# dayae1204/WeCLIP-ViT-CoMer

Hardware: AMD Instinct MI355X
Metric: images/sec (train fwd+bwd) ViT-B/16 512x512 VOC (higher is better)
Workload: dtype f16 MFMA operands / f32 accumulate, f32 residual+softmax+LN, PAR f32 arithmetic on 16-bit fixed-point affinities (precision=fast); 1 GPU; WeCLIP VOC full train step (the reference's model: frozen CLIP ViT-B/16 + adapters + decoder + GradCAM/affinity/PAR pseudo-labels), batch 16/GPU at 512x512, K=2 classes/image (BASELINE configs[2] without the ViT-CoMer inserts, for which the reference has no code); global_batch=16, parallelism=dp1

## Files before the change

### weclip-vit-comer_amd/csrc/par.hip

```cpp
#include "common.h"
#include <stdlib.h>

#define PAR_MAX_TAPS 64

struct ParTaps {
    int n;
    int dy[PAR_MAX_TAPS];
    int dx[PAR_MAX_TAPS];
    float pi[PAR_MAX_TAPS];
};

__device__ __forceinline__ int clampi(int v, int hi) { return v < 0 ? 0 : (v > hi ? hi : v); }

__global__ __launch_bounds__(256) void par_affinity_kernel(const float* __restrict__ img,
                                                            float* __restrict__ aff, int H, int W,
                                                            float w1, ParTaps taps) {
    const int x = blockIdx.x * 64 + (threadIdx.x & 63);
    const int y = blockIdx.y * 4 + (threadIdx.x >> 6);
    if (x >= W || y >= H) return;
    const long HW = (long)H * W;
    const float* I = img + (long)blockIdx.z * 3 * HW;
    const long p = (long)y * W + x;
    const float c0 = I[p], c1 = I[HW + p], c2 = I[2 * HW + p];
    const int T = taps.n;
    float s0 = 0.f, s1 = 0.f, s2 = 0.f;
    for (int t = 0; t < T; ++t) {
        const long o = (long)clampi(y + taps.dy[t], H - 1) * W + clampi(x + taps.dx[t], W - 1);
        s0 += I[o]; s1 += I[HW + o]; s2 += I[2 * HW + o];
    }
    const float m0 = s0 / T, m1 = s1 / T, m2 = s2 / T;
    float q0 = 0.f, q1 = 0.f, q2 = 0.f;
    for (int t = 0; t < T; ++t) {
        const long o = (long)clampi(y + taps.dy[t], H - 1) * W + clampi(x + taps.dx[t], W - 1);
        const float a = I[o] - m0, b = I[HW + o] - m1, c = I[2 * HW + o] - m2;
        q0 += a * a; q1 += b * b; q2 += c * c;
    }
    const float d0 = sqrtf(q0 / (T - 1)) + 1e-8f, d1 = sqrtf(q1 / (T - 1)) + 1e-8f,
                d2 = sqrtf(q2 / (T - 1)) + 1e-8f;
    float mx = -INFINITY, sum = 0.f;
    for (int t = 0; t < T; ++t) {
        const long o = (long)clampi(y + taps.dy[t], H - 1) * W + clampi(x + taps.dx[t], W - 1);
        const float a = fabsf(I[o] - c0) / d0 / w1, b = fabsf(I[HW + o] - c1) / d1 / w1,
                    c = fabsf(I[2 * HW + o] - c2) / d2 / w1;
        const float e = -(a * a + b * b + c * c) / 3.0f;
        const float nm = fmaxf(mx, e);
        sum = sum * __expf(mx - nm) + __expf(e - nm);
        mx = nm;
    }
    const float inv = 1.0f / sum;
    float* A = aff + (long)blockIdx.z * T * HW + p;
    for (int t = 0; t < T; ++t) {
        const long o = (long)clampi(y + taps.dy[t], H - 1) * W + clampi(x + taps.dx[t], W - 1);
        const float a = fabsf(I[o] - c0) / d0 / w1, b = fabsf(I[HW + o] - c1) / d1 / w1,
                    c = fabsf(I[2 * HW + o] - c2) / d2 / w1;
        const float e = -(a * a + b * b + c * c) / 3.0f;
        A[(long)t * HW] = __expf(e - mx) * inv + taps.pi[t];
    }
}

__device__ __forceinline__ long aff_base(bool tiled, long img, int T, int H, int W, int y, int x, long* tstride) {
    if (tiled) {
        const int XT = (W + 63) >> 6;
        *tstride = 64;
        return ((img * H + y) * XT + (x >> 6)) * (long)T * 64 + (x & 63);
    }
    *tstride = (long)H * W;
    return img * T * (long)H * W + (long)y * W + x;
}

#define PAR_Q_SLOTS(T_) ((T_) / 2 + 1)
template <int ND, bool TILED, bool H16 = false>
__global__ __launch_bounds__(256) void par_affinity_reg_kernel(const float* __restrict__ img,
                                                                float* __restrict__ aff, int H, int W,
                                                                float w1, ParTaps taps) {
    constexpr int T = 8 * ND;
    const int x = blockIdx.x * 64 + (threadIdx.x & 63);
    const int y = blockIdx.y * 4 + (threadIdx.x >> 6);
    if (x >= W || y >= H) return;
    const long HW = (long)H * W;
    const float* I = img + (long)blockIdx.z * 3 * HW;
    const long p = (long)y * W + x;
    const float c0 = I[p], c1 = I[HW + p], c2 = I[2 * HW + p];
    float v0[T], v1[T], v2[T];
    float s0 = 0.f, s1 = 0.f, s2 = 0.f;
    constexpr int RY[8] = {0, 0, 0, 1, 1, 2, 2, 2}, CX[8] = {0, 1, 2, 0, 2, 0, 1, 2};
#pragma unroll
    for (int dl = 0; dl < ND; ++dl) {
        const int d = taps.dx[8 * dl + 2];
        const int rw[3] = {clampi(y - d, H - 1) * W, y * W, clampi(y + d, H - 1) * W};
        const int cl[3] = {clampi(x - d, W - 1), x, clampi(x + d, W - 1)};
#pragma unroll
        for (int u = 0; u < 8; ++u) {
            const int t = 8 * dl + u;
            const int o = rw[RY[u]] + cl[CX[u]];
            v0[t] = I[o]; v1[t] = I[HW + o]; v2[t] = I[2 * HW + o];
            s0 += v0[t]; s1 += v1[t]; s2 += v2[t];
        }
    }
    const float m0 = s0 / T, m1 = s1 / T, m2 = s2 / T;
    float q0 = 0.f, q1 = 0.f, q2 = 0.f;
#pragma unroll
    for (int t = 0; t < T; ++t) {
        const float a = v0[t] - m0, b = v1[t] - m1, c = v2[t] - m2;
        q0 += a * a; q1 += b * b; q2 += c * c;
    }
    const float d0 = sqrtf(q0 / (T - 1)) + 1e-8f, d1 = sqrtf(q1 / (T - 1)) + 1e-8f,
                d2 = sqrtf(q2 / (T - 1)) + 1e-8f;
    const float r0 = 1.0f / (d0 * w1), r1 = 1.0f / (d1 * w1), r2 = 1.0f / (d2 * w1);
    float mx = -INFINITY;
#pragma unroll
    for (int t = 0; t < T; ++t) {
        const float a = fabsf(v0[t] - c0) * r0, b = fabsf(v1[t] - c1) * r1, c = fabsf(v2[t] - c2) * r2;
        v0[t] = -(a * a + b * b + c * c) * (1.0f / 3.0f);
        mx = fmaxf(mx, v0[t]);
    }
    float sum = 0.f;
#pragma unroll
    for (int t = 0; t < T; ++t) {
        v0[t] = __expf(v0[t] - mx);
        sum += v0[t];
    }
    const float inv = 1.0f / sum;
    if constexpr (H16) {
        const int XT = (W + 63) >> 6;
        unsigned* A2 = reinterpret_cast<unsigned*>(aff) + (((long)blockIdx.z * H + y) * XT + (x >> 6)) * (long)PAR_Q_SLOTS(T) * 64 + (x & 63);
        float amax = 0.f;
#pragma unroll
        for (int t = 0; t < T; ++t) {
            v0[t] = v0[t] * inv + taps.pi[t];
            amax = fmaxf(amax, v0[t]);
        }
        const float scale = amax * (1.0f / 65535.0f), rs = 65535.0f / amax;
        float carry = 0.f;
#pragma unroll
        for (int j = 0; j < T / 2; ++j) {
            const float a0 = v0[2 * j] + carry;
            const float q0 = fminf(fmaxf(rintf(a0 * rs), 0.f), 65535.f);
            carry = a0 - q0 * scale;
            const float a1 = v0[2 * j + 1] + carry;
            const float q1 = fminf(fmaxf(rintf(a1 * rs), 0.f), 65535.f);
            carry = a1 - q1 * scale;
            A2[j * 64] = (unsigned)q0 | ((unsigned)q1 << 16);
        }
        A2[(T / 2) * 64] = __float_as_uint(scale);
        return;
    }
    long ts;
    float* A = aff + aff_base(TILED, blockIdx.z, T, H, W, y, x, &ts);
#pragma unroll
    for (int t = 0; t < T; ++t) A[t * ts] = v0[t] * inv + taps.pi[t];
}

static void launch_affinity(const float* img, float* aff, int nb, int H, int W, const ParTaps& tp,
                            hipStream_t st, bool tiled, bool h16 = false) {
    dim3 grid(wc_cdiv(W, 64), wc_cdiv(H, 4), nb);
    const int pr = wc_prof_begin(st);
    if (tp.n == 48 && tiled && h16) {
        hipLaunchKernelGGL((par_affinity_reg_kernel<6, true, true>), grid, dim3(256), 0, st, img, aff, H, W, 0.3f, tp);
        wc_prof_end(pr, "par_affinity_reg_kernel<6, true, true>", 4.0 * nb * (double)H * W * 3 + nb * (double)H * W * (2.0 * tp.n + 4.0), st);
        return;
    }
    if (tp.n == 48 && tiled)
        hipLaunchKernelGGL((par_affinity_reg_kernel<6, true>), grid, dim3(256), 0, st, img, aff, H, W, 0.3f, tp);
    else if (tp.n == 48)
        hipLaunchKernelGGL((par_affinity_reg_kernel<6, false>), grid, dim3(256), 0, st, img, aff, H, W, 0.3f, tp);
    else
        hipLaunchKernelGGL(par_affinity_kernel, grid, dim3(256), 0, st, img, aff, H, W, 0.3f, tp);
    wc_prof_end(pr, tp.n == 48 ? (tiled ? "par_affinity_reg_kernel<6, true>" : "par_affinity_reg_kernel<6, false>") : "par_affinity_kernel",
                4.0 * nb * (double)H * W * (3 + tp.n), st);
}

#ifndef PAR_TAP_BATCH
#define PAR_TAP_BATCH 8
#endif
template <int CG, bool TILED, bool H16 = false, int ROWS = 4, int PAR_HALO = 4>
__global__ __launch_bounds__(64 * ROWS) void par_iter_kernel(const float* __restrict__ aff,
                                                        const float* __restrict__ min,
                                                        float* __restrict__ mout, int C, int H,
                                                        int W, ParTaps taps) {
    constexpr int TW = 64 + 2 * PAR_HALO, TH = ROWS + 2 * PAR_HALO;
    __shared__ float tile[H16 ? CG * TH * TW : 1];
    const int lx = threadIdx.x & 63, ly = threadIdx.x >> 6;
    int x = blockIdx.x * 64 + lx;
    int y = blockIdx.y * ROWS + ly;
    const bool live = x < W && y < H;
    if constexpr (H16) {
        x = x < W ? x : W - 1;
        y = y < H ? y : H - 1;
    } else {
        if (!live) return;
    }
    const long HW = (long)H * W;
    const long p = (long)y * W + x;
    const int T = taps.n;
    long ts;
    const float* A = aff + aff_base(TILED, blockIdx.z, T, H, W, y, x, &ts);
    const unsigned* A2 = reinterpret_cast<const unsigned*>(aff) +
                         (((long)blockIdx.z * H + y) * ((W + 63) >> 6) + (x >> 6)) * (long)PAR_Q_SLOTS(T) * 64 + (x & 63);
    float qscale = 1.f;
    if constexpr (H16) qscale = __uint_as_float(A2[(T / 2) * 64]);
    const float* M = min + (long)blockIdx.z * C * HW;
    float* O = mout + (long)blockIdx.z * C * HW + p;
    for (int cb = 0; cb < C; cb += CG) {
        float acc[CG];
        const float* Mc[CG];
#pragma unroll
        for (int k = 0; k < CG; ++k) {
            acc[k] = 0.f;
            Mc[k] = M + (long)(cb + k < C ? cb + k : C - 1) * HW;
        }
        if constexpr (H16) {
            if (cb) __syncthreads();
            for (int ty = ly; ty < TH; ty += ROWS) {
                const int ro = clampi(blockIdx.y * ROWS + ty - PAR_HALO, H - 1) * W;
                for (int tx = lx; tx < TW; tx += 64) {
                    const unsigned ob = (unsigned)(ro + clampi(blockIdx.x * 64 + tx - PAR_HALO, W - 1)) * 4u;
#pragma unroll
                    for (int k = 0; k < CG; ++k)
                        tile[(k * TH + ty) * TW + tx] = *reinterpret_cast<const float*>(reinterpret_cast<const char*>(Mc[k]) + ob);
                }
            }
            __syncthreads();
        }
        constexpr int TB_ = PAR_TAP_BATCH;
        int t = 0;
        for (; t + TB_ <= T; t += TB_) {
            float a[TB_], m[TB_][CG];
            unsigned a2[TB_ / 2];
            if constexpr (H16) {
#pragma unroll
                for (int u = 0; u < TB_ / 2; ++u) a2[u] = A2[((t >> 1) + u) * 64];
            }
            bool near = false;
            if constexpr (H16) near = (taps.dy[t] < 0 ? -taps.dy[t] : taps.dy[t]) <= PAR_HALO && (taps.dx[t] < 0 ? -taps.dx[t] : taps.dx[t]) <= PAR_HALO;
            if (near) {
                const int tb = (ly + PAR_HALO) * TW + lx + PAR_HALO;
#pragma unroll
                for (int u = 0; u < TB_; ++u) {
                    const int o = tb + (taps.dy[t + u] * TW + taps.dx[t + u]);
#pragma unroll
                    for (int k = 0; k < CG; ++k) m[u][k] = tile[k * TH * TW + o];
                }
            } else if constexpr (H16) {
                const int d = taps.dx[t + 2];
                const int rw[3] = {clampi(y - d, H - 1) * W, y * W, clampi(y + d, H - 1) * W};
                const int cl[3] = {clampi(x - d, W - 1), x, clampi(x + d, W - 1)};
                constexpr int RY[8] = {0, 0, 0, 1, 1, 2, 2, 2}, CX[8] = {0, 1, 2, 0, 2, 0, 1, 2};
                static_assert(TB_ == 8, "one batch = one dilation");
#pragma unroll
                for (int u = 0; u < TB_; ++u) {
                    const unsigned ob = (unsigned)(rw[RY[u]] + cl[CX[u]]) * 4u;
#pragma unroll
                    for (int k = 0; k < CG; ++k) m[u][k] = *reinterpret_cast<const float*>(reinterpret_cast<const char*>(Mc[k]) + ob);
                }
            } else {
#pragma unroll
                for (int u = 0; u < TB_; ++u) {
                    a[u] = A[(t + u) * ts];
                    const int o = clampi(y + taps.dy[t + u], H - 1) * W + clampi(x + taps.dx[t + u], W - 1);
#pragma unroll
                    for (int k = 0; k < CG; ++k) m[u][k] = Mc[k][o];
                }
            }
            if constexpr (H16) {
#pragma unroll
                for (int u = 0; u < TB_ / 2; ++u) {
                    a[2 * u] = (float)(a2[u] & 0xffffu);
                    a[2 * u + 1] = (float)(a2[u] >> 16);
                }
            }
#pragma unroll
            for (int u = 0; u < TB_; ++u)
#pragma unroll
                for (int k = 0; k < CG; ++k) acc[k] = fmaf(a[u], m[u][k], acc[k]);
        }
        for (; t < T; ++t) {
            const float a = A[t * ts];
            const int o = clampi(y + taps.dy[t], H - 1) * W + clampi(x + taps.dx[t], W - 1);
#pragma unroll
            for (int k = 0; k < CG; ++k) acc[k] = fmaf(a, Mc[k][o], acc[k]);
        }
#pragma unroll
        for (int k = 0; k < CG; ++k)
            if (cb + k < C && live) O[(long)(cb + k) * HW] = H16 ? acc[k] * qscale : acc[k];
    }
}

__global__ __launch_bounds__(256) void par_labels_kernel(const float* __restrict__ masks,
                                                          const long* __restrict__ valid_key,
                                                          const int* __restrict__ nch,
                                                          long* __restrict__ labels, int C, long HW) {
    const long p = (long)blockIdx.x * 256 + threadIdx.x;
    if (p >= HW) return;
    const int b = blockIdx.y;
    const int n = nch ? nch[b] : C;
    const float* M = masks + (long)b * C * HW + p;
    float best = M[0];
    int bi = 0;
    for (int c = 1; c < n; ++c) {
        const float v = M[(long)c * HW];
        if (v > best) { best = v; bi = c; }
    }
    labels[(long)b * HW + p] = valid_key[(long)b * C + bi];
}

static int build_taps(ParTaps* tp, const int* dilations, int n_dil, float w1, float w2) {
    if (!dilations || n_dil < 1 || n_dil * 8 > PAR_MAX_TAPS) return 1;
    static const int DY[8] = {-1, -1, -1, 0, 0, 1, 1, 1};
    static const int DX[8] = {-1, 0, 1, -1, 1, -1, 0, 1};
    const int T = n_dil * 8;
    float pos[PAR_MAX_TAPS];
    for (int d = 0; d < n_dil; ++d)
        for (int k = 0; k < 8; ++k) {
            const int t = d * 8 + k;
            tp->dy[t] = DY[k] * dilations[d];
            tp->dx[t] = DX[k] * dilations[d];
            pos[t] = (float)dilations[d] * ((DY[k] != 0 && DX[k] != 0) ? sqrtf(2.0f) : 1.0f);
        }
    float mean = 0.f;
    for (int t = 0; t < T; ++t) mean += pos[t];
    mean /= T;
    float var = 0.f;
    for (int t = 0; t < T; ++t) var += (pos[t] - mean) * (pos[t] - mean);
    const float sd = sqrtf(var / (T - 1)) + 1e-8f;
    float e[PAR_MAX_TAPS], mx = -INFINITY, sum = 0.f;
    for (int t = 0; t < T; ++t) {
        const float v = pos[t] / sd / w1;
        e[t] = -(v * v);
        mx = fmaxf(mx, e[t]);
    }
    for (int t = 0; t < T; ++t) sum += expf(e[t] - mx);
    for (int t = 0; t < T; ++t) tp->pi[t] = w2 * expf(e[t] - mx) / sum;
    tp->n = T;
    return 0;
}

extern "C" int wc_par_affinity(const float* img, float* aff, int B, int H, int W,
                               const int* dilations, int n_dil, void* stream) {
    WC_CHECK_ARG(img && aff && B > 0 && H > 0 && W > 0, "wc_par_affinity: bad argument");
    ParTaps tp;
    WC_CHECK_ARG(build_taps(&tp, dilations, n_dil, 0.3f, 0.01f) == 0, "wc_par_affinity: 1..8 dilations");
    launch_affinity(img, aff, B, H, W, tp, (hipStream_t)stream, false);
    WC_LAUNCH_CHECK("par_affinity_kernel");
    return WC_OK;
}

static const char* par_iter_name(int C, bool tiled, bool h16) {
    static const char* hn[3] = {"par_iter_kernel<2, true, true, 8, 12>", "par_iter_kernel<3, true, true, 8, 12>", "par_iter_kernel<4, true, true, 8, 12>"};
    static const char* names[2][3] = {{"par_iter_kernel<2, false>", "par_iter_kernel<3, false>", "par_iter_kernel<4, false>"},
                                      {"par_iter_kernel<2, true>", "par_iter_kernel<3, true>", "par_iter_kernel<4, true>"}};
    const int ci = C <= 2 ? 0 : (C == 3 ? 1 : 2);
    return h16 ? hn[ci] : names[tiled ? 1 : 0][ci];
}
static double par_iter_bytes(int B, int C, int H, int W, const ParTaps& tp, bool h16) {
    return h16 ? B * (double)H * W * (2.0 * tp.n + 4.0 + 8.0 * C) : 4.0 * B * (double)H * W * (tp.n + 2 * C);
}

static int launch_iter(const float* aff, const float* src, float* dst, int B, int C, int H, int W,
                       const ParTaps& tp, hipStream_t st, bool tiled, bool h16 = false, bool prof = true) {
    dim3 grid(wc_cdiv(W, 64), wc_cdiv(H, 4), B);
    if (h16) {
        const int pr = prof ? wc_prof_begin(st) : -1;
        dim3 grid8(wc_cdiv(W, 64), wc_cdiv(H, 8), B);
        if (C <= 2) hipLaunchKernelGGL((par_iter_kernel<2, true, true, 8, 12>), grid8, dim3(512), 0, st, aff, src, dst, C, H, W, tp);
        else if (C == 3) hipLaunchKernelGGL((par_iter_kernel<3, true, true, 8, 12>), grid8, dim3(512), 0, st, aff, src, dst, C, H, W, tp);
        else hipLaunchKernelGGL((par_iter_kernel<4, true, true, 8, 12>), grid8, dim3(512), 0, st, aff, src, dst, C, H, W, tp);
        wc_prof_end(pr, par_iter_name(C, tiled, true), par_iter_bytes(B, C, H, W, tp, true), st);
        WC_LAUNCH_CHECK("par_iter_kernel");
        return WC_OK;
    }
#define PAR_ITER_LAUNCH(CG_) \
    if (tiled) hipLaunchKernelGGL((par_iter_kernel<CG_, true>), grid, dim3(256), 0, st, aff, src, dst, C, H, W, tp); \
    else hipLaunchKernelGGL((par_iter_kernel<CG_, false>), grid, dim3(256), 0, st, aff, src, dst, C, H, W, tp);
    const int pr = prof ? wc_prof_begin(st) : -1;
    if (C <= 2) { PAR_ITER_LAUNCH(2) }
    else if (C == 3) { PAR_ITER_LAUNCH(3) }
    else { PAR_ITER_LAUNCH(4) }
    wc_prof_end(pr, par_iter_name(C, tiled, false), par_iter_bytes(B, C, H, W, tp, false), st);
    WC_LAUNCH_CHECK("par_iter_kernel");
    return WC_OK;
}

extern "C" int wc_par_iterate(const float* aff, const float* masks_in, float* masks_out, int B, int C,
                              int H, int W, const int* dilations, int n_dil, void* stream) {
    WC_CHECK_ARG(aff && masks_in && masks_out && masks_in != masks_out && B > 0 && C > 0 && H > 0 && W > 0,
                 "wc_par_iterate: bad argument (in-place not allowed)");
    ParTaps tp;
    WC_CHECK_ARG(build_taps(&tp, dilations, n_dil, 0.3f, 0.01f) == 0, "wc_par_iterate: 1..8 dilations");
    return launch_iter(aff, masks_in, masks_out, B, C, H, W, tp, (hipStream_t)stream, false);
}

static int par_forward_impl(const float* img, const float* masks, float* out, float* tmp, float* aff_ws, int B, int C,
                            int H, int W, const int* dilations, int n_dil, int num_iter, int group, void* stream, bool h16);

extern "C" int wc_par_forward(const float* img, const float* masks, float* out, float* tmp,
                              float* aff_ws, int B, int C, int H, int W, const int* dilations,
                              int n_dil, int num_iter, int group, void* stream) {
    return par_forward_impl(img, masks, out, tmp, aff_ws, B, C, H, W, dilations, n_dil, num_iter, group, stream, false);
}

extern "C" int wc_par_forward_h(const float* img, const float* masks, float* out, float* tmp,
                                float* aff_ws, int B, int C, int H, int W, const int* dilations,
                                int n_dil, int num_iter, int group, void* stream) {
    WC_CHECK_ARG(n_dil == 6, "wc_par_forward_h: needs 6 dilations (48 taps)");
    return par_forward_impl(img, masks, out, tmp, aff_ws, B, C, H, W, dilations, n_dil, num_iter, group, stream, true);
}

static int par_forward_impl(const float* img, const float* masks, float* out, float* tmp, float* aff_ws, int B, int C,
                            int H, int W, const int* dilations, int n_dil, int num_iter, int group, void* stream, bool h16) {
    WC_CHECK_ARG(img && masks && out && tmp && aff_ws && B > 0 && C > 0 && H > 0 && W > 0 &&
                     num_iter >= 1 && group >= 1,
                 "wc_par_forward: bad argument");
    WC_CHECK_ARG(out != masks && tmp != masks && out != tmp, "wc_par_forward: buffers must not alias");
    ParTaps tp;
    WC_CHECK_ARG(build_taps(&tp, dilations, n_dil, 0.3f, 0.01f) == 0, "wc_par_forward: 1..8 dilations");
    hipStream_t st = (hipStream_t)stream;
    const long HW = (long)H * W;
    const bool tiled = (tp.n == 48);
    for (int b0 = 0; b0 < B; b0 += group) {
        const int nb = (B - b0 < group) ? B - b0 : group;
        launch_affinity(img + (long)b0 * 3 * HW, aff_ws, nb, H, W, tp, st, tiled, h16 && tiled);
        WC_LAUNCH_CHECK("par_affinity_kernel");
        const float* src = masks + (long)b0 * C * HW;
        const int pr = wc_prof_begin_always(st);
        for (int i = 0; i < num_iter; ++i) {
            float* dst = (((num_iter - i) & 1) ? out : tmp) + (long)b0 * C * HW;
            int rc = launch_iter(aff_ws, src, dst, nb, C, H, W, tp, st, tiled, h16 && tiled, false);
            if (rc) return rc;
            src = dst;
        }
        wc_prof_end_n(pr, par_iter_name(C, tiled, h16 && tiled), num_iter * par_iter_bytes(nb, C, H, W, tp, h16 && tiled), st, num_iter);
    }
    return WC_OK;
}

extern "C" int wc_par_labels(const float* masks, const int64_t* valid_key, const int* nch,
                             int64_t* labels, int B, int C, int H, int W, void* stream) {
    WC_CHECK_ARG(masks && valid_key && labels && B > 0 && C > 0 && H > 0 && W > 0, "wc_par_labels: bad argument");
    const long HW = (long)H * W;
    dim3 grid(wc_cdiv(HW, 256), B);
    hipLaunchKernelGGL(par_labels_kernel, grid, dim3(256), 0, (hipStream_t)stream, masks,
                       (const long*)valid_key, nch, (long*)labels, C, HW);
    WC_LAUNCH_CHECK("par_labels_kernel");
    return WC_OK;
}
```

Baseline: 1276 images/sec.

## Restructure H16 PAR sweep with vectorized affinity I/O and register-cached taps

The affinity kernel now writes each dilation's four packed 16-bit pairs as one 128-bit store in a new strip layout. The H16 PAR iteration moves into a dedicated device function. It loads all packed affinities once per pixel as 128-bit vectors and keeps them in registers across channel groups. It also issues the halo-tile loads and the far-dilation gather before the barrier to overlap global latency, and adds an occupancy hint to launch bounds. The aim is fewer memory instructions and less stall time in the PAR iterations, at the cost of higher register pressure and reliance on asm barriers to steer the compiler.

Result: no change. 1289 images/sec, median of 6 (+1.0%).

```diff
diff --git a/weclip-vit-comer_amd/csrc/par.hip b/weclip-vit-comer_amd/csrc/par.hip
--- a/weclip-vit-comer_amd/csrc/par.hip
+++ b/weclip-vit-comer_amd/csrc/par.hip
@@ -69,6 +69,10 @@
 }
 
 #define PAR_Q_SLOTS(T_) ((T_) / 2 + 1)
+typedef unsigned par_u4 __attribute__((ext_vector_type(4)));
+__device__ __forceinline__ long par_strip(long img, int T, int H, int W, int y, int x) {
+    return ((img * H + y) * ((W + 63) >> 6) + (x >> 6)) * (long)PAR_Q_SLOTS(T) * 64;
+}
 template <int ND, bool TILED, bool H16 = false>
 __global__ __launch_bounds__(256) void par_affinity_reg_kernel(const float* __restrict__ img,
                                                                 float* __restrict__ aff, int H, int W,
@@ -122,8 +126,7 @@
     }
     const float inv = 1.0f / sum;
     if constexpr (H16) {
-        const int XT = (W + 63) >> 6;
-        unsigned* A2 = reinterpret_cast<unsigned*>(aff) + (((long)blockIdx.z * H + y) * XT + (x >> 6)) * (long)PAR_Q_SLOTS(T) * 64 + (x & 63);
+        unsigned* S = reinterpret_cast<unsigned*>(aff) + par_strip(blockIdx.z, T, H, W, y, x);
         float amax = 0.f;
 #pragma unroll
         for (int t = 0; t < T; ++t) {
@@ -133,16 +136,21 @@
         const float scale = amax * (1.0f / 65535.0f), rs = 65535.0f / amax;
         float carry = 0.f;
 #pragma unroll
-        for (int j = 0; j < T / 2; ++j) {
-            const float a0 = v0[2 * j] + carry;
-            const float q0 = fminf(fmaxf(rintf(a0 * rs), 0.f), 65535.f);
-            carry = a0 - q0 * scale;
-            const float a1 = v0[2 * j + 1] + carry;
-            const float q1 = fminf(fmaxf(rintf(a1 * rs), 0.f), 65535.f);
-            carry = a1 - q1 * scale;
-            A2[j * 64] = (unsigned)q0 | ((unsigned)q1 << 16);
-        }
-        A2[(T / 2) * 64] = __float_as_uint(scale);
+        for (int dl = 0; dl < ND; ++dl) {
+            unsigned w[4];
+#pragma unroll
+            for (int j = 0; j < 4; ++j) {
+                const float a0 = v0[8 * dl + 2 * j] + carry;
+                const float q0 = fminf(fmaxf(rintf(a0 * rs), 0.f), 65535.f);
+                carry = a0 - q0 * scale;
+                const float a1 = v0[8 * dl + 2 * j + 1] + carry;
+                const float q1 = fminf(fmaxf(rintf(a1 * rs), 0.f), 65535.f);
+                carry = a1 - q1 * scale;
+                w[j] = (unsigned)q0 | ((unsigned)q1 << 16);
+            }
+            reinterpret_cast<par_u4*>(S)[dl * 64 + (x & 63)] = par_u4{w[0], w[1], w[2], w[3]};
+        }
+        S[(T / 2) * 64 + (x & 63)] = __float_as_uint(scale);
         return;
     }
     long ts;
@@ -173,87 +181,162 @@
 #ifndef PAR_TAP_BATCH
 #define PAR_TAP_BATCH 8
 #endif
-template <int CG, bool TILED, bool H16 = false, int ROWS = 4, int PAR_HALO = 4>
-__global__ __launch_bounds__(64 * ROWS) void par_iter_kernel(const float* __restrict__ aff,
-                                                        const float* __restrict__ min,
-                                                        float* __restrict__ mout, int C, int H,
-                                                        int W, ParTaps taps) {
-    constexpr int TW = 64 + 2 * PAR_HALO, TH = ROWS + 2 * PAR_HALO;
-    __shared__ float tile[H16 ? CG * TH * TW : 1];
+__device__ __forceinline__ float par_ld(const float* base, unsigned ob) {
+    asm volatile("" : "+v"(ob));
+    return *reinterpret_cast<const float*>(reinterpret_cast<const char*>(base) + ob);
+}
+
+template <int CG, int ROWS, int HALO>
+__device__ __forceinline__ void par_sweep_h16(float* __restrict__ tile, const float* __restrict__ aff,
+                                              const float* __restrict__ min, float* __restrict__ mout, int C, int H,
+                                              int W, const ParTaps& taps) {
+    constexpr int ND = 6, TW = 64 + 2 * HALO, TH = ROWS + 2 * HALO, NR = TH / ROWS, W2 = TW - 64;
+    static_assert(TH % ROWS == 0 && W2 > 0 && W2 <= 64, "a thread fills TH / ROWS rows x 2 column pieces");
+    constexpr int RY[8] = {0, 0, 0, 1, 1, 2, 2, 2}, CX[8] = {0, 1, 2, 0, 2, 0, 1, 2};
     const int lx = threadIdx.x & 63, ly = threadIdx.x >> 6;
     int x = blockIdx.x * 64 + lx;
     int y = blockIdx.y * ROWS + ly;
     const bool live = x < W && y < H;
-    if constexpr (H16) {
-        x = x < W ? x : W - 1;
-        y = y < H ? y : H - 1;
-    } else {
-        if (!live) return;
-    }
+    x = x < W ? x : W - 1;
+    y = y < H ? y : H - 1;
     const long HW = (long)H * W;
-    const long p = (long)y * W + x;
-    const int T = taps.n;
-    long ts;
-    const float* A = aff + aff_base(TILED, blockIdx.z, T, H, W, y, x, &ts);
-    const unsigned* A2 = reinterpret_cast<const unsigned*>(aff) +
-                         (((long)blockIdx.z * H + y) * ((W + 63) >> 6) + (x >> 6)) * (long)PAR_Q_SLOTS(T) * 64 + (x & 63);
-    float qscale = 1.f;
-    if constexpr (H16) qscale = __uint_as_float(A2[(T / 2) * 64]);
     const float* M = min + (long)blockIdx.z * C * HW;
-    float* O = mout + (long)blockIdx.z * C * HW + p;
+    float* O = mout + (long)blockIdx.z * C * HW + (long)y * W + x;
+
+    int dil[ND], ff = ND, dff = 0;
+#pragma unroll
+    for (int dl = ND - 1; dl >= 0; --dl) {
+        dil[dl] = taps.dx[8 * dl + 2];
+        if ((dil[dl] < 0 ? -dil[dl] : dil[dl]) > HALO) { ff = dl; dff = dil[dl]; }
+    }
+    auto gather = [&](int d, const float* const (&Mc)[CG], float (&g)[8][CG]) {
+        const int rw[3] = {clampi(y - d, H - 1) * W, y * W, clampi(y + d, H - 1) * W};
+        const int cl[3] = {clampi(x - d, W - 1), x, clampi(x + d, W - 1)};
+#pragma unroll
+        for (int u = 0; u < 8; ++u) {
+            const unsigned ob = (unsigned)(rw[RY[u]] + cl[CX[u]]) * 4u;
+#pragma unroll
+            for (int k = 0; k < CG; ++k) g[u][k] = par_ld(Mc[k], ob);
+        }
+    };
+    unsigned fo[NR][2];
+    {
+        const int c0 = clampi(blockIdx.x * 64 + lx - HALO, W - 1);
+        const int c1 = clampi(blockIdx.x * 64 + 64 + (lx < W2 ? lx : W2 - 1) - HALO, W - 1);
+#pragma unroll
+        for (int r = 0; r < NR; ++r) {
+            const int ro = clampi(blockIdx.y * ROWS + ly + r * ROWS - HALO, H - 1) * W;
+            fo[r][0] = (unsigned)(ro + c0) * 4u;
+            fo[r][1] = (unsigned)(ro + c1) * 4u;
+        }
+    }
+    const unsigned* S = reinterpret_cast<const unsigned*>(aff) + par_strip(blockIdx.z, 8 * ND, H, W, y, x);
+    par_u4 q[ND];
+    float qscale = 0.f;
+    int tb = (ly + HALO) * TW + lx + HALO;
     for (int cb = 0; cb < C; cb += CG) {
+        asm volatile("" : "+v"(x), "+v"(y), "+v"(tb));
+        const float* Mc[CG];
+#pragma unroll
+        for (int k = 0; k < CG; ++k) Mc[k] = M + (long)(cb + k < C ? cb + k : C - 1) * HW;
+        float fv[NR][2][CG], g[8][CG];
+#pragma unroll
+        for (int r = 0; r < NR; ++r)
+#pragma unroll
+            for (int h = 0; h < 2; ++h)
+#pragma unroll
+                for (int k = 0; k < CG; ++k) fv[r][h][k] = par_ld(Mc[k], fo[r][h]);
+        if (cb == 0) {
+#pragma unroll
+            for (int dl = 0; dl < ND; ++dl) q[dl] = reinterpret_cast<const par_u4*>(S)[dl * 64 + (x & 63)];
+            qscale = __uint_as_float(S[4 * ND * 64 + (x & 63)]);
+        }
+        gather(dff, Mc, g);
+        if (cb) __syncthreads();
+#pragma unroll
+        for (int r = 0; r < NR; ++r)
+#pragma unroll
+            for (int k = 0; k < CG; ++k) {
+                float* row = tile + (k * TH + ly + r * ROWS) * TW + lx;
+                row[0] = fv[r][0][k];
+                if (lx < W2) row[64] = fv[r][1][k];
+            }
+        __syncthreads();
         float acc[CG];
-        const float* Mc[CG];
-#pragma unroll
-        for (int k = 0; k < CG; ++k) {
-            acc[k] = 0.f;
-            Mc[k] = M + (long)(cb + k < C ? cb + k : C - 1) * HW;
-        }
-        if constexpr (H16) {
-            if (cb) __syncthreads();
-            for (int ty = ly; ty < TH; ty += ROWS) {
-                const int ro = clampi(blockIdx.y * ROWS + ty - PAR_HALO, H - 1) * W;
-                for (int tx = lx; tx < TW; tx += 64) {
-                    const unsigned ob = (unsigned)(ro + clampi(blockIdx.x * 64 + tx - PAR_HALO, W - 1)) * 4u;
-#pragma unroll
-                    for (int k = 0; k < CG; ++k)
-                        tile[(k * TH + ty) * TW + tx] = *reinterpret_cast<const float*>(reinterpret_cast<const char*>(Mc[k]) + ob);
+#pragma unroll
+        for (int k = 0; k < CG; ++k) acc[k] = 0.f;
+#pragma unroll
+        for (int dl = 0; dl < ND; ++dl) {
+            const bool near = (dil[dl] < 0 ? -dil[dl] : dil[dl]) <= HALO;
+            const unsigned a2[4] = {q[dl].x, q[dl].y, q[dl].z, q[dl].w};
+            auto fma8 = [&](const float (&m)[8][CG]) {
+#pragma unroll
+                for (int u = 0; u < 8; ++u) {
+                    const float a = (u & 1) ? (float)(a2[u >> 1] >> 16) : (float)(a2[u >> 1] & 0xffffu);
+#pragma unroll
+                    for (int k = 0; k < CG; ++k) acc[k] = fmaf(a, m[u][k], acc[k]);
                 }
-            }
-            __syncthreads();
-        }
-        constexpr int TB_ = PAR_TAP_BATCH;
-        int t = 0;
-        for (; t + TB_ <= T; t += TB_) {
-            float a[TB_], m[TB_][CG];
-            unsigned a2[TB_ / 2];
-            if constexpr (H16) {
-#pragma unroll
-                for (int u = 0; u < TB_ / 2; ++u) a2[u] = A2[((t >> 1) + u) * 64];
-            }
-            bool near = false;
-            if constexpr (H16) near = (taps.dy[t] < 0 ? -taps.dy[t] : taps.dy[t]) <= PAR_HALO && (taps.dx[t] < 0 ? -taps.dx[t] : taps.dx[t]) <= PAR_HALO;
+            };
             if (near) {
-                const int tb = (ly + PAR_HALO) * TW + lx + PAR_HALO;
-#pragma unroll
-                for (int u = 0; u < TB_; ++u) {
-                    const int o = tb + (taps.dy[t + u] * TW + taps.dx[t + u]);
+                float m[8][CG];
+#pragma unroll
+                for (int u = 0; u < 8; ++u) {
+                    const int o = tb + dil[dl] * ((RY[u] - 1) * TW + (CX[u] - 1));
 #pragma unroll
                     for (int k = 0; k < CG; ++k) m[u][k] = tile[k * TH * TW + o];
                 }
-            } else if constexpr (H16) {
-                const int d = taps.dx[t + 2];
-                const int rw[3] = {clampi(y - d, H - 1) * W, y * W, clampi(y + d, H - 1) * W};
-                const int cl[3] = {clampi(x - d, W - 1), x, clampi(x + d, W - 1)};
-                constexpr int RY[8] = {0, 0, 0, 1, 1, 2, 2, 2}, CX[8] = {0, 1, 2, 0, 2, 0, 1, 2};
-                static_assert(TB_ == 8, "one batch = one dilation");
-#pragma unroll
-                for (int u = 0; u < TB_; ++u) {
-                    const unsigned ob = (unsigned)(rw[RY[u]] + cl[CX[u]]) * 4u;
-#pragma unroll
-                    for (int k = 0; k < CG; ++k) m[u][k] = *reinterpret_cast<const float*>(reinterpret_cast<const char*>(Mc[k]) + ob);
-                }
+                fma8(m);
+            } else if (dl == ff) {
+                fma8(g);
             } else {
+                float m[8][CG];
+                gather(dil[dl], Mc, m);
+                fma8(m);
+            }
+#pragma unroll
+            for (int k = 0; k < CG; ++k) asm volatile("" : "+v"(acc[k]));
+        }
+#pragma unroll
+        for (int k = 0; k < CG; ++k)
+            if (cb + k < C && live) O[(long)(cb + k) * HW] = acc[k] * qscale;
+    }
+}
+
+#ifndef PAR_SWEEP_WAVES
+#define PAR_SWEEP_WAVES 4
+#endif
+template <int CG, bool TILED, bool H16 = false, int ROWS = 4, int PAR_HALO = 4>
+__global__ __launch_bounds__(64 * ROWS, H16 ? PAR_SWEEP_WAVES : 0) void par_iter_kernel(const float* __restrict__ aff,
+                                                        const float* __restrict__ min,
+                                                        float* __restrict__ mout, int C, int H,
+                                                        int W, ParTaps taps) {
+    if constexpr (H16) {
+        __shared__ float tile[CG * (ROWS + 2 * PAR_HALO) * (64 + 2 * PAR_HALO)];
+        par_sweep_h16<CG, ROWS, PAR_HALO>(tile, aff, min, mout, C, H, W, taps);
+    } else {
+        const int lx = threadIdx.x & 63, ly = threadIdx.x >> 6;
+        const int x = blockIdx.x * 64 + lx;
+        const int y = blockIdx.y * ROWS + ly;
+        if (x >= W || y >= H) return;
+        const long HW = (long)H * W;
+        const long p = (long)y * W + x;
+        const int T = taps.n;
+        long ts;
+        const float* A = aff + aff_base(TILED, blockIdx.z, T, H, W, y, x, &ts);
+        const float* M = min + (long)blockIdx.z * C * HW;
+        float* O = mout + (long)blockIdx.z * C * HW + p;
+        for (int cb = 0; cb < C; cb += CG) {
+            float acc[CG];
+            const float* Mc[CG];
+#pragma unroll
+            for (int k = 0; k < CG; ++k) {
+                acc[k] = 0.f;
+                Mc[k] = M + (long)(cb + k < C ? cb + k : C - 1) * HW;
+            }
+            constexpr int TB_ = PAR_TAP_BATCH;
+            int t = 0;
+            for (; t + TB_ <= T; t += TB_) {
+                float a[TB_], m[TB_][CG];
 #pragma unroll
                 for (int u = 0; u < TB_; ++u) {
                     a[u] = A[(t + u) * ts];
@@ -261,28 +344,21 @@
 #pragma unroll
                     for (int k = 0; k < CG; ++k) m[u][k] = Mc[k][o];
                 }
+#pragma unroll
+                for (int u = 0; u < TB_; ++u)
+#pragma unroll
+                    for (int k = 0; k < CG; ++k) acc[k] = fmaf(a[u], m[u][k], acc[k]);
             }
-            if constexpr (H16) {
-#pragma unroll
-                for (int u = 0; u < TB_ / 2; ++u) {
-                    a[2 * u] = (float)(a2[u] & 0xffffu);
-                    a[2 * u + 1] = (float)(a2[u] >> 16);
-                }
+            for (; t < T; ++t) {
+                const float a = A[t * ts];
+                const int o = clampi(y + taps.dy[t], H - 1) * W + clampi(x + taps.dx[t], W - 1);
+#pragma unroll
+                for (int k = 0; k < CG; ++k) acc[k] = fmaf(a, Mc[k][o], acc[k]);
             }
 #pragma unroll
-            for (int u = 0; u < TB_; ++u)
-#pragma unroll
-                for (int k = 0; k < CG; ++k) acc[k] = fmaf(a[u], m[u][k], acc[k]);
-        }
-        for (; t < T; ++t) {
-            const float a = A[t * ts];
-            const int o = clampi(y + taps.dy[t], H - 1) * W + clampi(x + taps.dx[t], W - 1);
-#pragma unroll
-            for (int k = 0; k < CG; ++k) acc[k] = fmaf(a, Mc[k][o], acc[k]);
-        }
-#pragma unroll
-        for (int k = 0; k < CG; ++k)
-            if (cb + k < C && live) O[(long)(cb + k) * HW] = H16 ? acc[k] * qscale : acc[k];
+            for (int k = 0; k < CG; ++k)
+                if (cb + k < C) O[(long)(cb + k) * HW] = acc[k];
+        }
     }
 }
 
```
